# pyxploiter/HandMvNet

Measured on AMD Instinct MI355X. Metric: samples/sec (BxV frames) eval_fps.py, 8-view 256x256; 21-kpt L2 vs reference, higher is better.
Workload: dtype f32; 1 GPU; BASELINE configs[2]: B=32/GPU x V=8 x 256x256, resnet50_paper backbone, d=524, cross_attn x5, GCN decoder; global_batch=32, views=8, frame=256, parallelism=sample-shard x1

## Files before the change

### handmvnet_amd/csrc/conv_igemm.hip

```cpp
#include <cstdio>
#include <cstdlib>
#include <cstring>
#include <type_traits>

#include "kernels.h"

namespace hmv {

typedef float f32x16 __attribute__((ext_vector_type(16)));
typedef float f32x4 __attribute__((ext_vector_type(4)));
typedef _Float16 f16x8 __attribute__((ext_vector_type(8)));
typedef _Float16 f16x4 __attribute__((ext_vector_type(4)));


#ifndef HMV_UB
#define HMV_UB 4
#endif
#ifndef HMV_UB_F16
#define HMV_UB_F16 4
#endif
#ifndef HMV_TOUT
#define HMV_TOUT 1
#endif

// ... 939 lines not shown
                            _Float16 *op = reinterpret_cast<_Float16 *>(outv) + orow[u] * p.ldc + col;
                            if constexpr (W == 8)
                                *reinterpret_cast<f16x8 *>(op) = f16x8{(_Float16)t[0][0], (_Float16)t[0][1], (_Float16)t[0][2], (_Float16)t[0][3],
                                                                       (_Float16)t[W4 - 1][0], (_Float16)t[W4 - 1][1], (_Float16)t[W4 - 1][2], (_Float16)t[W4 - 1][3]};
                            else
                                *reinterpret_cast<f16x4 *>(op) = f16x4{(_Float16)t[0][0], (_Float16)t[0][1], (_Float16)t[0][2], (_Float16)t[0][3]};
                        } else {
#pragma unroll
                            for (int q = 0; q < W4; ++q)
                                *reinterpret_cast<f32x4 *>(reinterpret_cast<float *>(outv) + orow[u] * p.ldc + col + 4 * q) = t[q];
                        }
                    }
                }
            };
            bool wide = false;
            if constexpr (F16 && !GENERIC && BN % 8 == 0 && (NT % (BN / 8)) == 0)
                wide = (p.out_f16 || p.out_split) && ((p.out_split ? p.ldc >> 1 : p.ldc) & 7) == 0 &&
                       (p.res == nullptr || ((p.res_split ? p.ldr >> 1 : p.ldr) & 7) == 0);
            if constexpr (F16 && !GENERIC && BN % 8 == 0 && (NT % (BN / 8)) == 0) {
                if (wide) drain(std::integral_constant<int, 8>{});
                else drain(std::integral_constant<int, 4>{});
            } else {
                drain(std::integral_constant<int, 4>{});
            }
            }
        } else if (GENERIC) {
            for (int idx = tid; idx < SR * BN; idx += NT) {
                const int sr = idx / BN, c = idx - sr * BN;
                const int m = mt * BM + tile_row(sr), col = n0 + c;
                if (m >= p.M || col >= p.Cout) continue;
                const size_t orow = p.scatter ? out_row(m) : (size_t)m;
                const size_t rrow = p.rg_out ? (size_t)(m / p.rg_out) * p.rg_in + (m % p.rg_out) : (size_t)m;
                float v = sC[sr * LDC + c] + p.bias[col];
                if (p.res) v += p.res_f16 ? (float)reinterpret_cast<const _Float16 *>(p.res)[rrow * p.ldr + col]
                                          : reinterpret_cast<const float *>(p.res)[rrow * p.ldr + col];
                if (p.act == ACT_RELU) v = v > 0.f ? v : 0.f;
                else if (p.act == ACT_GELU) v = 0.5f * v * (1.f + erff(v * 0.70710678118654752440f));
                else if (p.act == ACT_LEAKY) v = v > 0.f ? v : 0.01f * v;
                if (p.out_f16) reinterpret_cast<_Float16 *>(outv)[orow * p.ldc + col] = (_Float16)v;
                else reinterpret_cast<float *>(outv)[orow * p.ldc + col] = v;
            }
        }
    }
    if (p.dbg && tid == 0) {
        unsigned hwid, xcc;
        asm volatile("s_getreg_b32 %0, hwreg(HW_REG_HW_ID)" : "=s"(hwid));
        asm volatile("s_getreg_b32 %0, hwreg(HW_REG_XCC_ID)" : "=s"(xcc));
        unsigned long long *d = p.dbg + 8 * (size_t)blockIdx.x;
        d[0] = t1c - t0c; d[1] = t1r - t0r; d[2] = t_entry; d[3] = t0r; d[4] = t1r;
        d[5] = __builtin_amdgcn_s_memrealtime(); d[6] = hwid; d[7] = xcc;
    }
}

int conv_tile_bn(ConvTile t) {
    switch (t) {
        case TILE_128x32: return 32;
        case TILE_128x64: case TILE_64x64: return 64;
        case TILE_128x256: case TILE_256x256: case TILE_128x256_K16: case TILE_256x256_RING: return 256;
        default: return 128;
    }
}

static const char *kTileShape[TILE_COUNT] = {"128x32", "128x64", "128x128", "256x128", "128x256", "256x256", "128x128,k16",
                                              "128x256,k16", "256x128,k16", "64x64", "256x128,k16,w8", "256x256,ring"};
static const char *tile_name(const char *dtype, ConvTile t, int mode, bool partn = false, bool rd = false) {
    static char names[2][TILE_COUNT][3][3][56];
    if (t < 0 || t >= TILE_COUNT || mode < 0 || mode > 2) return "conv_igemm<?>";
    const int d = dtype[1] == '1';
    char *n = names[d][t][mode][rd ? 2 : (partn ? 1 : 0)];
    if (!n[0])
        snprintf(n, sizeof(names[0][0][0][0]), "conv_igemm_%s<%s,%s%s>", dtype, kTileShape[t],
                 mode == 0 ? "taps" : (mode == 1 ? "1x1" : "dense"), rd ? ",rowsum" : (partn ? ",skipN" : ""));
    return n;
}
const char *conv_tile_name_f16(ConvTile t, int mode) {
    return tile_name("f16", t, mode);
}
const char *conv_tile_name(ConvTile t, int mode) { return tile_name("f32", t, mode); }

ConvTile conv_dense_tile(ConvTile t, bool f16) {
    switch (t) {
        case TILE_128x32: case TILE_128x64: case TILE_64x64: case TILE_256x128: return t;
        case TILE_256x128_K16: case TILE_256x256: case TILE_256x256_RING: return TILE_256x128;
        default: return TILE_128x128;
    }
}
bool conv_partial_n(ConvTile t, int Cout) {
    if (t != TILE_128x128 && t != TILE_256x128 && t != TILE_256x256) return false;
    const int bn = conv_tile_bn(t);
    return (Cout + bn - 1) / bn * bn - Cout >= 32;
}

ConvTile conv_pick_tile(int M, int Cout, int K, bool f16, bool has_res) {
    static const int forced = HMV_DEV_INT("HMV_FORCE_TILE", -1);
    static const bool force_all = HMV_DEV_ENV("HMV_FORCE_TILE_ALL") != nullptr;
    if ((Cout > 64 || force_all) && forced >= 0 && forced < TILE_COUNT) return (ConvTile)forced;
    if (!f16 && Cout >= 256 && K <= 128 && M >= 65536) return TILE_128x128_K16;
    static const bool no_w8 = HMV_DEV_ENV("HMV_NO_W8") != nullptr;
    if (!no_w8 && !f16 && has_res && K <= 256 && Cout >= 512 && (long long)((M + 255) / 256) * ((Cout + 127) / 128) >= 2048)
        return TILE_256x128_K16W8;
    if (!no_w8 && !f16 && !has_res && K >= 256 && K <= 512 && Cout == 128 && (long long)((M + 255) / 256) >= 1024)
        return TILE_256x128_K16W8;
    if (!f16 && Cout > 64 && Cout <= 192 && Cout % 64 != 0 && M >= 16384 && K < 2048) return TILE_128x32;
    if (!f16 && Cout > 256 && Cout % 128 != 0 && Cout % 128 <= 64 && M >= 16384 && (long long)((M + 127) / 128) * ((Cout + 63) / 64) < 1024)
        return TILE_64x64;
    if (Cout > 128 && Cout <= 192 && M >= 16384) return (M + 255) / 256 >= 256 ? TILE_256x256 : TILE_128x64;
    if (Cout > 256 && M >= 16384 && Cout % 128 != 0 && Cout % 128 <= 64) return TILE_128x64;
    if (Cout > 128 && (long long)((M + 255) / 256) * ((Cout + 255) / 256) >= 512) return TILE_256x256;
    if (Cout > 64 && (long long)((M + 255) / 256) * ((Cout + 127) / 128) >= 512) return TILE_256x128;
    if (!f16 && K >= 2048 && Cout >= 256 && (long long)((M + 127) / 128) * ((Cout + 127) / 128) < 256 &&
        (long long)((M + 127) / 128) * ((Cout + 63) / 64) >= 256)
        return TILE_128x64;
    if (Cout > 32 && (long long)((M + 127) / 128) * ((Cout + 127) / 128) < 256) return TILE_64x64;
    if (!f16 && K <= 256 && Cout >= 256 && (long long)((M + 127) / 128) * ((Cout + 127) / 128) < 1024) return TILE_64x64;
    if (Cout > 64) return TILE_128x128;
    if (Cout > 32) return TILE_128x64;
    return TILE_128x32;
}

template <typename T, int BM, int BN, int WGM, int WGN, int MODE, bool GENERIC, int KB, bool PARTN = false, bool RD = false, bool X3 = false, bool C32 = false>
static hipError_t launch_one(ConvParams p, hipStream_t s) {
    if constexpr (!X3 && sizeof(T) == 2 && KB == 64 && !GENERIC && !PARTN && !RD && MODE != MODE_HALO) {
        if (p.x3_plane) return launch_one<T, BM, BN, WGM, WGN, MODE, GENERIC, KB, PARTN, RD, true>(p, s);
    }
    constexpr bool tout = HMV_TOUT && sizeof(T) == 2 && !GENERIC && !RD;
    constexpr int ns = ring_stages(sizeof(T) == 2, KB, GENERIC, RD, BM, BN);
    const size_t lds = MODE == MODE_HALO ? (size_t)2 * (HALO_ROWS + BN) * KB * sizeof(T) + 256
                                         : (size_t)lds_floats(BM, BN, WGM, KB * (int)sizeof(T) / 4, RD, !tout, ns) * sizeof(float) + (tout ? 256 : 0);
    auto kern = conv_igemm<T, BM, BN, WGM, WGN, MODE, GENERIC, KB, PARTN, RD, X3, C32>;
    static DeviceOnce once;
    if (const hipError_t e = once.run([&](int) { return set_max_lds(lds, kern); }); e != hipSuccess) return e;
    p.mtiles = (p.M + BM - 1) / BM;
    p.ntiles = (p.Cout + BN - 1) / BN;
    if (p.mtiles * p.ntiles < 4 * p.stagger_blocks) p.stagger = 0;
    hipLaunchKernelGGL(kern, dim3(p.mtiles * p.ntiles * (p.ksl > 1 ? p.ksl : 1) * (p.phases > 1 ? p.phases : 1)), dim3(64 * WGM * WGN), lds, s, p);
    return hipGetLastError();
}

template <typename T, int BM, int BN, int WGM, int WGN, int KB>
static hipError_t launch_modes(const ConvParams &p, bool one, bool generic, hipStream_t s) {
    if (generic) return one ? launch_one<T, BM, BN, WGM, WGN, MODE_1X1, true, KB>(p, s) : launch_one<T, BM, BN, WGM, WGN, MODE_TAPS, true, KB>(p, s);
    return one ? launch_one<T, BM, BN, WGM, WGN, MODE_1X1, false, KB>(p, s) : launch_one<T, BM, BN, WGM, WGN, MODE_TAPS, false, KB>(p, s);
}
template <typename T, int BM, int BN, int WGM, int WGN, int KB>
static hipError_t launch_plain(const ConvParams &p, bool one, hipStream_t s) {
    return one ? launch_one<T, BM, BN, WGM, WGN, MODE_1X1, false, KB>(p, s) : launch_one<T, BM, BN, WGM, WGN, MODE_TAPS, false, KB>(p, s);
}

hipError_t launch_conv(ConvParams p, ConvTile tile, hipStream_t s, const char **name, const ConvRoute &route) {
    if (name) *name = "conv_igemm<none>";
    if (p.M <= 0) return hipSuccess;
    {
        float *page = nullptr;
        hipError_t e = ensure_zero_page(&page);
        if (e != hipSuccess) return e;
        p.zero = page;
    }
    if (!p.lda) p.lda = p.Cin;
    if (!p.ldw) p.ldw = p.Kpad;
    {
        struct Stagger { int ticks = 0, blocks = 256, mode = 0; };
        static const Stagger st = [] {
            Stagger r;
            if (const char *e = HMV_DEV_ENV("HMV_STAGGER")) {
                r.ticks = atoi(e);
                const char *c = strchr(e, ',');
                if (c) { r.blocks = atoi(c + 1); c = strchr(c + 1, ','); if (c) r.mode = atoi(c + 1); }
            }
            return r;
        }();
        p.stagger = st.ticks;
        p.stagger_blocks = st.blocks;
        p.stagger_mode = st.mode;
        static const int pf = HMV_DEV_INT("HMV_PREFETCH", 0);
        p.prefetch = pf;
        static const int burst = HMV_DEV_INT("HMV_BURST", 1);
        p.burst = burst;
    }
    p.acc_scale = ldexpf(1.f, -p.acc_shift);
    bool generic = p.scatter || p.rg_out || p.act == ACT_GELU || p.act == ACT_LEAKY || (p.ldc & 3) ||
                   (p.res && (p.ldr & 3));
    if (HMV_TOUT && p.in_f16 && (p.out_f16 || p.out_split) &&
        (((p.out_split ? p.ldc >> 1 : p.ldc) & 7) || (p.res && ((p.res_split ? p.ldr >> 1 : p.ldr) & 7))))
        generic = true;
    if (p.phases > 1 && (p.phases != 4 || !p.scatter || p.R != 2 || p.S != 2 || p.stride != 1 || p.ksl > 1 || p.in2 || p.rd_cout || p.phase_stride == 0))
        return hipErrorInvalidValue;
    const bool one = p.R == 1 && p.S == 1 && p.pad_h == 0 && p.pad_w == 0;
    if (p.nx_wgt && (generic || p.tall || !conv_stream_chain_ok(p, p.nx_cout, route))) return hipErrorInvalidValue;
    if (p.pool && (generic || p.tall || !conv_hs_supported(p, route))) return hipErrorInvalidValue;
// ... 31 lines not shown
                    tile == TILE_128x256_K16 || tile == TILE_256x128_K16))
        tile = TILE_128x128;
    const int ch = p.in_f16 ? 64 : 32, epc = p.in_f16 ? 8 : 4;
    const bool dense = p.Cin % ch != 0;
    if (p.x3_plane && (!p.in_f16 || generic || p.rd_cout || p.cwrap || p.x3_plane % 8 != 0 || p.Cin != 2 * p.x3_plane ||
                       (!dense && p.x3_plane % 32 != 0) || tile == TILE_128x128_K16 || tile == TILE_128x256_K16 || tile == TILE_256x128_K16 || tile == TILE_256x256_RING))
        return hipErrorInvalidValue;
    if ((p.cwrap || p.res_split || p.out_split || p.acc_shift) &&
        (!p.in_f16 || p.rd_cout || (p.ldc & 3) || (p.res && (p.ldr & 3)) || p.act == ACT_GELU || p.act == ACT_LEAKY))
        return hipErrorInvalidValue;
    if (p.rd_cout && !generic && conv_rds_supported(p, route)) return launch_conv_rds(p, s, name);
    if (p.rd_cout) {
        if (generic || p.R != 3 || p.S != 1 || p.stride != 1 || p.pad_h != 1 || p.pad_w != 0 || p.Cout != 3 * p.rd_cout || p.Cout > 256 ||
            (p.rd_cout & 3) || (p.ldc & 3) || (p.res && (p.ldr & 3)) || 128 % p.Wo != 0 || p.Ho != p.H || p.Wo != p.W)
            return hipErrorInvalidValue;
        if (dense) {
            if (p.Cin % epc != 0 || p.lda % epc != 0 || p.Kpad > (1 << 16)) return hipErrorInvalidValue;
            p.cpt = p.Cin / epc;
            p.cpt_magic = p.cpt > 1 ? (unsigned)(0xFFFFFFFFu / (unsigned)p.cpt) + 1u : 0u;
            p.s_magic = 0u;
        }
        const bool wide = p.Cout > 128;
        if (name) *name = tile_name(p.in_f16 ? "f16" : "f32", wide ? TILE_128x256 : TILE_128x128, dense ? 2 : 0, false, true);
#define HMV_RD(T_, KB_)                                                                                                  \
        if (wide) return dense ? launch_one<T_, 128, 256, 2, 4, MODE_DENSE, false, KB_, false, true>(p, s)                  \
                               : launch_one<T_, 128, 256, 2, 4, MODE_TAPS, false, KB_, false, true>(p, s);                  \
        return dense ? launch_one<T_, 128, 128, 2, 2, MODE_DENSE, false, KB_, false, true>(p, s)                            \
                     : launch_one<T_, 128, 128, 2, 2, MODE_TAPS, false, KB_, false, true>(p, s);
        if (p.in_f16) { HMV_RD(_Float16, 64) }
        HMV_RD(float, 32)
#undef HMV_RD
    }
    if (dense) {
        if (p.Cin % epc != 0 || p.lda % epc != 0 || generic || p.Kpad > (1 << 16)) return hipErrorInvalidValue;
        p.cpt = (p.x3_plane ? p.x3_plane : p.Cin) / epc;
        p.cpt_magic = p.cpt > 1 ? (unsigned)(0xFFFFFFFFu / (unsigned)p.cpt) + 1u : 0u;
        p.s_magic = p.S > 1 ? (unsigned)(0xFFFFFFFFu / (unsigned)p.S) + 1u : 0u;
        if (p.up && (p.R != 1 || p.S != 1 || p.pad_h || p.pad_w || p.stride != 1)) return hipErrorInvalidValue;
        tile = conv_dense_tile(tile, p.in_f16 != 0);
    }
    static const int ring = HMV_DEV_INT("HMV_F16_RING", 0);
    if (ring && p.in_f16 && tile == TILE_256x256 && !generic && !dense && !p.x3_plane && !p.cwrap && !p.rd_cout && p.ksl <= 1)
        tile = TILE_256x256_RING;
    static const bool halo = HMV_DEV_ENV("HMV_NO_HALO") == nullptr;
    const bool use_halo = halo && p.in_f16 && (tile == TILE_256x256 || tile == TILE_256x128) && !generic && !dense && !p.x3_plane && !p.cwrap && !p.rd_cout &&
                          p.ksl <= 1 && !p.in2 && !p.res && !p.up && p.R == 3 && p.S == 3 && p.stride == 1 && p.pad_h == 1 && p.pad_w == 1 &&
                          p.Ho == p.H && p.Wo == p.W && p.H % 16 == 0 && p.W % 16 == 0 && p.Cin % 64 == 0 && p.lda == p.Cin &&
                          p.M % 256 == 0;
    if (use_halo) {
        if (name) *name = tile == TILE_256x256 ? "conv_igemm_f16<256x256,halo>" : "conv_igemm_f16<256x128,halo>";
        return tile == TILE_256x256 ? launch_one<_Float16, 256, 256, 2, 4, MODE_HALO, false, 64>(p, s)
                                    : launch_one<_Float16, 256, 128, 4, 2, MODE_HALO, false, 64>(p, s);
    }
    const int mode = dense ? MODE_DENSE : (one ? MODE_1X1 : MODE_TAPS);
    static const int no_skip = HMV_DEV_INT("HMV_NO_SKIPN", 0);
    const bool partn = !no_skip && !p.in_f16 && !generic && conv_partial_n(tile, p.Cout) && !(dense && tile == TILE_256x256);
    if (name) *name = p.in_f16 ? conv_tile_name_f16(tile, mode) : tile_name("f32", tile, mode, partn);
    if (partn) {
#define HMV_PARTN(BM_, BN_, WGM_, WGN_)                                                                              \
        switch (mode) {                                                                                                 \
            case MODE_DENSE: return launch_one<float, BM_, BN_, WGM_, WGN_, MODE_DENSE, false, 32, true>(p, s);         \
            case MODE_1X1: return launch_one<float, BM_, BN_, WGM_, WGN_, MODE_1X1, false, 32, true>(p, s);             \
            default: return launch_one<float, BM_, BN_, WGM_, WGN_, MODE_TAPS, false, 32, true>(p, s);                  \
        }
        if (tile == TILE_128x128) { HMV_PARTN(128, 128, 2, 2) }
        if (tile == TILE_256x128) { HMV_PARTN(256, 128, 4, 2) }
        if (tile == TILE_256x256) { HMV_PARTN(256, 256, 2, 4) }
#undef HMV_PARTN
    }
    if (dense) {
        if (p.in_f16) {
            static const bool no192 = HMV_DEV_ENV("HMV_NO_N192") != nullptr;
            if (tile == TILE_256x128 && p.Cout > 128 && p.Cout <= 192 && !generic && !no192) {
                if (name) *name = "conv_igemm_f16<256x192,dense>";
                return launch_one<_Float16, 256, 192, 4, 2, MODE_DENSE, false, 64>(p, s);
            }
            switch (tile) {
                case TILE_128x32: return launch_one<_Float16, 128, 32, 4, 1, MODE_DENSE, false, 64>(p, s);
                case TILE_128x64: return launch_one<_Float16, 128, 64, 2, 2, MODE_DENSE, false, 64>(p, s);
                case TILE_64x64: return launch_one<_Float16, 64, 64, 2, 2, MODE_DENSE, false, 64>(p, s);
                case TILE_256x128: return launch_one<_Float16, 256, 128, 4, 2, MODE_DENSE, false, 64>(p, s);
                default: return launch_one<_Float16, 128, 128, 2, 2, MODE_DENSE, false, 64>(p, s);
            }
        }
        switch (tile) {
            case TILE_128x32: return launch_one<float, 128, 32, 4, 1, MODE_DENSE, false, 32>(p, s);
            case TILE_128x64: return launch_one<float, 128, 64, 2, 2, MODE_DENSE, false, 32>(p, s);
            case TILE_64x64: return launch_one<float, 64, 64, 2, 2, MODE_DENSE, false, 32>(p, s);
            case TILE_256x128: return launch_one<float, 256, 128, 4, 2, MODE_DENSE, false, 32>(p, s);
            default: return launch_one<float, 128, 128, 2, 2, MODE_DENSE, false, 32>(p, s);
        }
    }
    if (p.in_f16) {
        switch (tile) {
            case TILE_128x32: return launch_modes<_Float16, 128, 32, 4, 1, 64>(p, one, generic, s);
            case TILE_128x64: return launch_modes<_Float16, 128, 64, 2, 2, 64>(p, one, generic, s);
            case TILE_64x64: return launch_modes<_Float16, 64, 64, 2, 2, 64>(p, one, generic, s);
            case TILE_128x128: return launch_modes<_Float16, 128, 128, 2, 2, 64>(p, one, generic, s);
            case TILE_128x128_K16: return launch_plain<_Float16, 128, 128, 2, 2, 32>(p, one, s);
            case TILE_256x128: return launch_plain<_Float16, 256, 128, 4, 2, 64>(p, one, s);
            case TILE_128x256: return launch_plain<_Float16, 128, 256, 2, 4, 64>(p, one, s);
            case TILE_256x128_K16: return launch_plain<_Float16, 256, 128, 4, 2, 32>(p, one, s);
            case TILE_128x256_K16: return launch_plain<_Float16, 128, 256, 2, 4, 32>(p, one, s);
            case TILE_256x256: return launch_plain<_Float16, 256, 256, 2, 4, 64>(p, one, s);
            case TILE_256x256_RING: return launch_plain<_Float16, 256, 256, 2, 4, 32>(p, one, s);
            default: return hipErrorInvalidValue;
        }
    }
    switch (tile) {
        case TILE_128x32: return launch_modes<float, 128, 32, 4, 1, 32>(p, one, generic, s);
        case TILE_128x64: {
            static const bool no25664 = HMV_DEV_ENV("HMV_NO_T256x64") != nullptr;
            if (!no25664 && !generic && !one && p.Cout == 64 && p.M >= 524288) {
                if (name) *name = "conv_igemm_f32<256x64,taps>";
                return launch_plain<float, 256, 64, 4, 2, 32>(p, false, s);
            }
            return launch_modes<float, 128, 64, 2, 2, 32>(p, one, generic, s);
        }
        case TILE_128x128: return launch_modes<float, 128, 128, 2, 2, 32>(p, one, generic, s);
        case TILE_256x128: return launch_plain<float, 256, 128, 4, 2, 32>(p, one, s);
        case TILE_128x256: return launch_plain<float, 128, 256, 2, 4, 32>(p, one, s);
        case TILE_256x256: return launch_plain<float, 256, 256, 2, 4, 32>(p, one, s);
        case TILE_128x128_K16: return launch_plain<float, 128, 128, 2, 2, 16>(p, one, s);
        case TILE_128x256_K16: return launch_plain<float, 128, 256, 2, 2, 16>(p, one, s);
        case TILE_256x128_K16: return launch_plain<float, 256, 128, 2, 2, 16>(p, one, s);
        case TILE_64x64: return launch_modes<float, 64, 64, 2, 2, 32>(p, one, generic, s);
        case TILE_256x128_K16W8: return launch_plain<float, 256, 128, 4, 2, 16>(p, one, s);
        default: return hipErrorInvalidValue;
    }
}

}
```

### handmvnet_amd/csrc/engine.hip

```cpp
#include <hip/hip_runtime.h>

#include <algorithm>
#include <array>
#include <cmath>
#include <cstdarg>
#include <cstdio>
#include <cstdlib>
#include <cstring>
#include <map>
#include <string>
#include <vector>

#include "../../include/handmv.h"
#include "kernels.h"

using namespace hmv;

namespace {

constexpr int NJ = 21, HEADS = 8, DHEAD = 128, INNER = HEADS * DHEAD;
constexpr int DHEAD_LQ = 256, INNER_LQ = HEADS * DHEAD_LQ;
const int kBlocks[3][4] = {{2, 2, 2, 2}, {3, 4, 6, 3}, {3, 4, 6, 3}};
const int kHrChannels[2][4] = {{40, 80, 160, 320}, {64, 128, 256, 512}};
inline int cpad(int c) { return (c + 3) / 4 * 4; }
// ... 2155 lines not shown
    eng.host["w"] = wt;
    bt.shape = {Cout};
    bt.data.assign(Cout, 0.f);
    if (bias_host) bt.data.assign(bias_host, bias_host + Cout);
    if (rd) {
        HostTensor g1 = bt, m0 = bt, v1 = bt;
        g1.data.assign(Cout, 1.f); m0.data.assign(Cout, 0.f);
        v1.data.assign(Cout, 1.f - 1e-5f);
        eng.host["bn.weight"] = g1; eng.host["bn.bias"] = bt; eng.host["bn.running_mean"] = m0; eng.host["bn.running_var"] = v1;
    } else if (bias_host) {
        eng.host["b"] = bt;
    }
    Loader L{&eng};
    L.split = dtype == HMV_F32X3;
    Layer layer;
    L.conv(layer, "op", "w", bias_host && !rd ? "b" : "", rd ? "bn" : "", Cout, Cin, R, S, 0, half, rd, nullptr, tall);
    int rc = L.rc;
    if (rc == HMV_OK && rd && !layer.rd_cout) { eng.err = "the layer was not packed row-decomposed"; rc = HMV_ERR_ARG; }
    const int Ho = (H + 2 * pad - R) / stride + 1, Wo = (W + 2 * pad - S) / stride + 1;
    const void *x = in, *res = residual;
    void *din = nullptr, *dres = nullptr;
    hipError_t e = hipSuccess;
    if (rc == HMV_OK && half) {
        const int mode = dtype == HMV_F32X3 ? 2 : 1;
        const size_t rows_in = (size_t)N * H * W, rows_out = (size_t)N * Ho * Wo;
        e = hipMalloc(&din, rows_in * Cin * 2 * mode);
        if (e == hipSuccess && residual) e = hipMalloc(&dres, rows_out * Cout * 2 * mode);
        if (e == hipSuccess) e = launch_rows_f32_to_half(in, din, rows_in, Cin, mode, s);
        if (e == hipSuccess && residual) e = launch_rows_f32_to_half(residual, dres, rows_out, Cout, mode, s);
        x = din;
        res = dres;
    }
    if (rc == HMV_OK && e == hipSuccess) {
        Arena dummy;
        Runner Rn{&eng, s, false, HMV_OK, dummy};
        Rn.kernel_name = kernel_name;
        Rn.route = route;
        Rn.conv(layer, static_cast<const float *>(x), N, H, W, stride, pad, pad, static_cast<float *>(out), Cout, static_cast<const float *>(res),
                Cout, relu ? ACT_RELU : ACT_NONE, Ho, Wo, 0, 0, 0, 0, 0, out16);
        rc = Rn.rc;
        if (rc == HMV_OK) e = hipStreamSynchronize(s);
    }
    if (din) (void)hipFree(din);
    if (dres) (void)hipFree(dres);
    for (void *ptr : eng.dev_allocs) (void)hipFree(ptr);
    if (rc != HMV_OK) { g_create_err = std::string(who) + ": " + eng.err; return rc; }
    if (e != hipSuccess) { g_create_err = std::string(who) + ": " + hipGetErrorString(e); return HMV_ERR_HIP; }
    return HMV_OK;
}

static ConvRoute route_sel(int sel) {
    ConvRoute r = conv_rule();
    if (sel) r.stream = sel == 2 ? ROUTE_FORCE : ROUTE_NEVER;
    return r;
}
static ConvRoute route_f16(int sel) {
    ConvRoute r = conv_rule();
    if (sel) r.stream = r.gemm8 = r.hs = (sel == 2 || sel == 8) ? ROUTE_FORCE : ROUTE_NEVER;
    if (sel >= 3 && sel <= 7) r.ht = (sel == 4 || sel == 6) ? ROUTE_NEVER : ROUTE_FORCE;
    r.ht_m16 = sel != 5 && sel != 6;
    r.ht_persist = sel == 7 ? 2 : (sel == 3 ? 0 : 1);
    r.gemm8_persist = sel == 8 ? 2 : (sel == 2 ? 0 : 1);
    return r;
}
static ConvRoute route_x3(int sel) {
    ConvRoute r = conv_rule();
    if (sel) r.x3k16 = sel == 2 ? ROUTE_FORCE : ROUTE_NEVER;
    return r;
}
static ConvRoute route_rd(int sel) {
    ConvRoute r = conv_rule();
    if (sel) r.rds = sel == 2 ? ROUTE_FORCE : ROUTE_NEVER;
    return r;
}

extern "C" {

int hmv_op_conv2d(int32_t device, const float *in, int32_t N, int32_t H, int32_t W, int32_t Cin, const float *w_oihw,
                  const float *bias_host, int32_t Cout, int32_t R, int32_t S, int32_t stride, int32_t pad, const float *residual,
                  int32_t relu, float *out, void *stream) {
    return op_conv("hmv_op_conv2d", device, HMV_F32, in, N, H, W, Cin, w_oihw, bias_host, Cout, R, S, stride, pad, residual, relu, out, false,
                   conv_rule(), nullptr, stream);
}

int hmv_op_conv2d_ex(int32_t device, int32_t dtype, const float *in, int32_t N, int32_t H, int32_t W, int32_t Cin, const float *w_oihw,
                     const float *bias_host, int32_t Cout, int32_t R, int32_t S, int32_t stride, int32_t pad, const float *residual,
                     int32_t relu, float *out, void *stream) {
    return op_conv("hmv_op_conv2d_ex", device, dtype, in, N, H, W, Cin, w_oihw, bias_host, Cout, R, S, stride, pad, residual, relu, out, false,
                   conv_rule(), nullptr, stream);
}

int hmv_op_conv2d_sel(int32_t device, const float *in, int32_t N, int32_t H, int32_t W, int32_t Cin, const float *w_oihw, const float *bias_host,
                      int32_t Cout, int32_t R, int32_t S, int32_t stride, int32_t pad, const float *residual, int32_t relu, float *out,
                      int32_t kernel_sel, const char **kernel_name, void *stream) {
    if (kernel_sel < 0 || kernel_sel > 2) { g_create_err = "hmv_op_conv2d_sel: kernel_sel must be 0, 1 or 2"; return HMV_ERR_ARG; }
    return op_conv("hmv_op_conv2d_sel", device, HMV_F32, in, N, H, W, Cin, w_oihw, bias_host, Cout, R, S, stride, pad, residual, relu, out, false,
                   route_sel(kernel_sel), kernel_name, stream);
}

int hmv_op_conv2d_f16(int32_t device, const float *in, int32_t N, int32_t H, int32_t W, int32_t Cin, const float *w_oihw, const float *bias_host,
                      int32_t Cout, int32_t R, int32_t S, int32_t stride, int32_t pad, const float *residual, int32_t relu, void *out_f16,
                      int32_t kernel_sel, const char **kernel_name, void *stream) {
    if (kernel_sel < 0 || kernel_sel > 8) { g_create_err = "hmv_op_conv2d_f16: kernel_sel must be 0 .. 8"; return HMV_ERR_ARG; }
    return op_conv("hmv_op_conv2d_f16", device, HMV_F16, in, N, H, W, Cin, w_oihw, bias_host, Cout, R, S, stride, pad, residual, relu, out_f16,
                   true, route_f16(kernel_sel), kernel_name, stream, kernel_sel >= 3 && kernel_sel <= 7);
}

int hmv_op_conv2d_x3(int32_t device, const float *in, int32_t N, int32_t H, int32_t W, int32_t Cin, const float *w_oihw, const float *bias_host,
                     int32_t Cout, int32_t R, int32_t S, int32_t stride, int32_t pad, const float *residual, int32_t relu, float *out,
                     int32_t kernel_sel, const char **kernel_name, void *stream) {
    if (kernel_sel < 0 || kernel_sel > 2) { g_create_err = "hmv_op_conv2d_x3: kernel_sel must be 0, 1 or 2"; return HMV_ERR_ARG; }
    return op_conv("hmv_op_conv2d_x3", device, HMV_F32X3, in, N, H, W, Cin, w_oihw, bias_host, Cout, R, S, stride, pad, residual, relu, out, false,
                   route_x3(kernel_sel), kernel_name, stream);
}

int hmv_op_conv2d_rd(int32_t device, const float *in, int32_t N, int32_t H, int32_t W, int32_t C, const float *w_oihw, const float *bias_host,
                     const float *residual, int32_t relu, float *out, int32_t kernel_sel, const char **kernel_name, void *stream) {
    if (!in || !w_oihw || !out || C % 4 != 0 || 3 * C > 256 || C % 32 == 0 || W <= 0 || 128 % W != 0 || kernel_sel < 0 || kernel_sel > 2) {
        g_create_err = "hmv_op_conv2d_rd: C % 4 == 0, C % 32 != 0, 3 C <= 256, 128 % W == 0, kernel_sel 0 .. 2";
        return HMV_ERR_ARG;
    }
    return op_conv("hmv_op_conv2d_rd", device, HMV_F32, in, N, H, W, C, w_oihw, bias_host, C, 3, 3, 1, 1, residual, relu, out, false,
                   route_rd(kernel_sel), kernel_name, stream, false, true);
}

}

extern "C" int hmv_op_hr_fuse_up(int32_t device, int32_t f16, const float *base, int32_t N, int32_t H, int32_t W, int32_t C, int32_t nsrc,
                                 const float *const *src, const int32_t *src_c, const int32_t *shift, const float *const *w_host,
                                 const float *const *bias_host, int32_t relu, void *out, void *stream) {
    if (!base || !out || !src || !src_c || !shift || !w_host || !bias_host || nsrc < 1 || nsrc > 3 || N <= 0 || H <= 0 || W <= 0 || C <= 0) {
        g_create_err = "hmv_op_hr_fuse_up: bad arguments";
        return HMV_ERR_ARG;
    }
    if (hipSetDevice(device) != hipSuccess) { g_create_err = "hipSetDevice failed"; return HMV_ERR_HIP; }
    hipStream_t s = static_cast<hipStream_t>(stream);
    HrFuseParams p{};
    p.N = N; p.H = H; p.W = W; p.C = C; p.ldc = C; p.nsrc = nsrc; p.relu = relu ? 1 : 0; p.f16 = f16 ? 1 : 0;
    std::vector<void *> owned;
    auto fail = [&](int rc, const std::string &msg) {
        for (void *q : owned) (void)hipFree(q);
        g_create_err = "hmv_op_hr_fuse_up: " + msg;
        return rc;
    };
    hipError_t e = hipSuccess;
    auto dev_copy = [&](const std::vector<float> &v) -> float * {
        void *d = nullptr;
        if (e == hipSuccess) e = hipMalloc(&d, v.size() * sizeof(float));
// ... 34 lines not shown
```

### handmvnet_amd/csrc/kernels.h

```cpp
#pragma once
#include <hip/hip_runtime.h>
#include <stdint.h>
#include <stdlib.h>

#include <atomic>
#include <mutex>

#ifdef HMV_DEV_KNOBS
#define HMV_DEV_ENV(name) getenv(name)
#else
#define HMV_DEV_ENV(name) (static_cast<const char *>(nullptr))
#endif
#define HMV_DEV_INT(name, dflt) (HMV_DEV_ENV(name) ? atoi(HMV_DEV_ENV(name)) : (dflt))

namespace hmv {

enum Act { ACT_NONE = 0, ACT_RELU = 1, ACT_GELU = 2, ACT_LEAKY = 3 };

class DeviceOnce {
    std::atomic<bool> done_[64] = {};
    std::mutex m_;
public:
    template <typename F>
    hipError_t run(F &&body, int *dev_out = nullptr) {
// ... 35 lines not shown
    int scatter;
    int osy, osx, ooy, oox;
    int mtiles, ntiles;
    const float *zero;
    int cpt;
    unsigned cpt_magic, s_magic;
    int cwrap;
    int res_split;
    int x3_plane;
    int acc_shift;
    float acc_scale;
    int out_split;
    int ngroup;
    int m16;
    int tall;
    int rd_cout;
    const void *in2;
    int ksplit, H2, W2, lda2, stride2;
    int lda;
    int ldw;
    int ksl, kslice;
    size_t out_slice;
    int phases;
    size_t phase_stride;
    int burst;
    int prefetch;
    int stagger;
    int stagger_mode;
    int stagger_blocks;
    unsigned long long *dbg;
    int pool, pool_h, pool_w;
    const void *nx_wgt;
    const float *nx_bias;
    void *nx_out;
    int nx_cout, nx_ldw, nx_ldc, nx_act;
};

enum ConvTile { TILE_128x32 = 0, TILE_128x64 = 1, TILE_128x128 = 2, TILE_256x128 = 3, TILE_128x256 = 4, TILE_256x256 = 5,
                TILE_128x128_K16 = 6, TILE_128x256_K16 = 7, TILE_256x128_K16 = 8, TILE_64x64 = 9,
                TILE_256x128_K16W8 = 10,
                TILE_256x256_RING = 11,
                TILE_COUNT = 12 };
int conv_tile_bn(ConvTile t);
const char *conv_tile_name(ConvTile t, int mode);
const char *conv_tile_name_f16(ConvTile t, int mode);
ConvTile conv_pick_tile(int M, int Cout, int K, bool f16 = false, bool has_res = false);
ConvTile conv_dense_tile(ConvTile t, bool f16);
bool conv_partial_n(ConvTile t, int Cout);

enum { ROUTE_RULE = -1, ROUTE_NEVER = 0, ROUTE_FORCE = 1 };
struct ConvRoute {
    int stream = ROUTE_RULE, gemm8 = ROUTE_RULE, hs = ROUTE_RULE, rds = ROUTE_RULE, ht = ROUTE_RULE, x3k16 = ROUTE_RULE;
    int gemm8_persist = 1, ht_persist = 1;
    int ht_m16 = 1;
};
inline const ConvRoute &conv_rule() {
    static const ConvRoute r = [] {
        ConvRoute q;
        if (HMV_DEV_ENV("HMV_NO_STREAM")) q.stream = ROUTE_NEVER;
        if (HMV_DEV_ENV("HMV_NO_GEMM8")) q.gemm8 = ROUTE_NEVER;
        if (HMV_DEV_ENV("HMV_NO_HS")) q.hs = ROUTE_NEVER;
        if (HMV_DEV_ENV("HMV_NO_RDS")) q.rds = ROUTE_NEVER;
        return q;
    }();
    return r;
}

hipError_t launch_conv(ConvParams p, ConvTile tile, hipStream_t s, const char **name = nullptr, const ConvRoute &route = conv_rule());
bool conv_stream_supported(const ConvParams &p, const ConvRoute &route = conv_rule());
bool conv_stream_chain_ok(const ConvParams &p, int nx_cout, const ConvRoute &route = conv_rule());
hipError_t launch_conv_stream(const ConvParams &p, hipStream_t s, const char **name);

hipError_t launch_nchw_to_nhwc4(const float *x, float *out, int N, int H, int W, hipStream_t s);
hipError_t launch_maxpool3s2(const float *in, float *out, int N, int H, int W, int C, int Ho, int Wo, hipStream_t s);
hipError_t launch_soft_argmax(const float *hm, int ld, int N, int h, int w, float *coords, float *crop_img,
                              float image_size, float heatmap_size, float *hm_nchw, hipStream_t s);
hipError_t launch_sample_gather(const float *feat, int N, int H, int W, int C, const float *coords, float *out,
                                hipStream_t s, int elem_bytes = 4);
hipError_t launch_nchw_to_nhwc8_f16(const float *x, void *out, int N, int H, int W, hipStream_t s);
hipError_t launch_frames_to_input(const uint8_t *frames, const int *boxes, int N, int Hf, int Wf, int S_h, int S_w, const float *mean,
                                  const float *std, int out_mode, void *out, hipStream_t s, bool s2d = false);
hipError_t launch_nchw_to_s2d(const float *x, void *out, int N, int H, int W, int mode, hipStream_t s);
hipError_t launch_nchw_to_nhwc_split(const float *x, void *out, int N, int H, int W, hipStream_t s);
hipError_t launch_maxpool3s2_split(const void *in, void *out, int N, int H, int W, int C, int Ho, int Wo, hipStream_t s);
hipError_t launch_nhwc_split_to_nchw(const void *in, float *out, int N, int H, int W, int C, hipStream_t s);
hipError_t launch_rows_f32_to_half(const float *in, void *out, size_t rows, int C, int mode, hipStream_t s);
hipError_t launch_maxpool3s2_f16(const void *in, void *out, int N, int H, int W, int C, int Ho, int Wo, hipStream_t s);
hipError_t launch_nhwc_f16_to_nchw(const void *in, float *out, int N, int H, int W, int C, hipStream_t s);
hipError_t launch_sample_blend(const float *s4, int lds4, int C, int N, int H, int W, const float *coords,
                               float *tokens, int ldt, int col0, hipStream_t s);
hipError_t launch_tokens_finalize(float *tokens, int ldt, int d, int fdim, int N, int V, const float *coords,
                                  const float *bbox, const float *intr, int pos_mask, const float *pe,
                                  float *raw_copy, hipStream_t s, void *pairs = nullptr);
hipError_t launch_layernorm(const float *x, int ldx, int rows, int d, const float *g1, const float *b1, float *y,
                            int ldy, const float *g2, const float *b2, float *y2, hipStream_t s);
hipError_t launch_attention(const float *qkv, int B, int T, int Tq, int koff, int Tk, float *out, hipStream_t s, int pairs = 0, int x3 = 0);
hipError_t launch_attention_d256(const float *q, int q_ld, int q_bstride, const float *k, const float *v, int kv_ld, int B, int T,
                                 int Tq, float *out, hipStream_t s, int pairs = 0);
hipError_t launch_add_pe(const float *x, int ldx, int rows, int T, int d, const float *pe, float *y, int ldy, hipStream_t s);
hipError_t launch_splitk_layernorm(const float *slab, int S, int rows, int lds, int d, const float *bias, const float *res, int ldr,
                                   int rg_out, int rg_in, const float *g1, const float *b1, float *y, int ldy, const float *g2,
                                   const float *b2, float *y2, hipStream_t s);
hipError_t launch_splitk_reduce(const float *slab, int S, int rows, int lds, int N, const float *bias, const float *res, int ldr,
                                int rg_out, int rg_in, int act, float *out, int ldc, hipStream_t s);
hipError_t launch_cheb_mix(const float *y, int ldy, int B, int co, const float *tk, const float *bias, int leaky,
                           float *out, int ldo, hipStream_t s);
// ... 59 lines not shown
```

Baseline: 6023 frames/s.

## Add persistent f32 256x256 implicit-GEMM conv kernel with epilogue/prologue overlap

Adds a persistent-grid f32 256x256 implicit-GEMM conv kernel launched with at most one block per CU. Blocks walk tiles in an XCD-aware order and start the next tile's global-to-LDS loads before storing the last epilogue pass of the current tile. It replaces the plain 256x256 f32 launch when the shape qualifies, there is no residual, and there are at least twice as many tiles as CUs. The aim is to hide per-tile prologue and epilogue latency and cut block launch overhead, at the cost of more complex wait-count logic and possible load imbalance when tiles do not divide evenly across CUs.

```diff
diff --git a/handmvnet_amd/csrc/conv_igemm.hip b/handmvnet_amd/csrc/conv_igemm.hip
--- a/handmvnet_amd/csrc/conv_igemm.hip
+++ b/handmvnet_amd/csrc/conv_igemm.hip
@@ -1015,6 +1015,240 @@
     }
 }
 
+template <int MODE>
+__global__ __launch_bounds__(512, 2) void conv_igemm32p(const ConvParams p) {
+    constexpr int BM = 256, BN = 256, WGM = 2, WGN = 4, KB = 32, NT = 64 * WGM * WGN;
+    constexpr int LPR = KB / 4, RPW = 64 / LPR, RPS = NT / LPR, NQ = LPR / 2;
+    constexpr int WM = BM / WGM, WN = BN / WGN, TM = WM / 32, TN = WN / 32, AP = BM / RPS, BP = BN / RPS, LDC = BN + 4;
+    constexpr int AS = stage_blocks(BM, BN, WGM, KB), SR = WGM * AS * 32, NPS = TM / AS;
+    constexpr int TPR = BN / 4, RPP = NT / TPR, NPASS = SR / RPP;
+    constexpr int NST = NPASS;
+    static_assert(MODE == MODE_1X1 || MODE == MODE_TAPS, "chunked modes");
+    static_assert(TM % AS == 0 && SR * LDC <= lds_floats(BM, BN, WGM, KB) && SR % RPP == 0 && AP + BP + NST < 64, "epilogue shape / vmcnt range");
+    extern __shared__ __attribute__((aligned(16))) float smem[];
+    float *sA = smem, *sB = smem + 2 * BM * KB;
+
+    const int tid = threadIdx.x, lane = tid & 63;
+    const int wave = __builtin_amdgcn_readfirstlane(tid >> 6);
+    const int l31 = lane & 31, kh = lane >> 5;
+    const int wm = wave / WGN, wn = wave % WGN;
+    const int lrow = tid / LPR, kqs = (tid & 7) ^ ((tid >> 4) & 7), koff = 4 * kqs;
+    const float *zero = p.zero;
+    const int HoWo = p.Ho * p.Wo, nk = p.Kpad / KB, ntile = p.mtiles * p.ntiles;
+    auto tile_of = [&](int v, int &mt_, int &nt_) {
+        const int xcd = v & 7, loc = v >> 3, q = ntile >> 3, r = ntile & 7;
+        const int lid = (xcd < r ? xcd * (q + 1) : r * (q + 1) + (xcd - r) * q) + loc;
+        mt_ = lid / p.ntiles;
+        nt_ = lid - mt_ * p.ntiles;
+    };
+
+    const float *aptr[AP], *wptr[BP];
+    int astep[AP], hi0[AP], wi0[AP];
+    int dmt = 0, cr = 0, cs = 0, cc = 0, cdelta = 0, ck = 0;
+    auto setup = [&](int mt_, int nt_) {
+        dmt = mt_;
+        cr = cs = cc = cdelta = ck = 0;
+#pragma unroll
+        for (int i = 0; i < AP; ++i) {
+            const int m = mt_ * BM + i * RPS + lrow;
+            const bool ok = m < p.M;
+            const int mm = ok ? m : 0;
+            const int n = mm / HoWo, rem = mm - n * HoWo;
+            const int ho = rem / p.Wo, wo = rem - ho * p.Wo;
+            const float *base = reinterpret_cast<const float *>(p.in) + (size_t)n * p.H * p.W * p.lda;
+            hi0[i] = ok ? ho * p.stride - p.pad_h : -(1 << 28);
+            wi0[i] = wo * p.stride - p.pad_w;
+            if constexpr (MODE == MODE_1X1) {
+                aptr[i] = ok ? base + (hi0[i] * p.W + wi0[i]) * p.lda + koff : zero;
+                astep[i] = ok ? KB : 0;
+            } else {
+                aptr[i] = base + (ok ? (hi0[i] * p.W + wi0[i]) * p.lda + koff : 0);
+                astep[i] = 0;
+            }
+        }
+#pragma unroll
+        for (int i = 0; i < BP; ++i) wptr[i] = reinterpret_cast<const float *>(p.wgt) + (size_t)(nt_ * BN + i * RPS + lrow) * p.ldw + 4 * kqs;
+    };
+#define HMV_P_DMA(buf)                                                                                      \
+    {                                                                                                       \
+        _Pragma("unroll") for (int i = 0; i < AP; ++i) {                                                    \
+            const float *src_;                                                                              \
+            if constexpr (MODE == MODE_1X1) {                                                               \
+                src_ = aptr[i];                                                                             \
+                aptr[i] += astep[i];                                                                        \
+            } else {                                                                                        \
+                const bool ok_ = (unsigned)(hi0[i] + cr) < (unsigned)p.H && (unsigned)(wi0[i] + cs) < (unsigned)p.W; \
+                src_ = ok_ ? aptr[i] + cdelta : zero;                                                       \
+            }                                                                                               \
+            HMV_GLDS16(src_, sA + ((buf) * BM + i * RPS + wave * RPW) * KB);                                \
+        }                                                                                                   \
+        _Pragma("unroll") for (int i = 0; i < BP; ++i) {                                                    \
+            HMV_GLDS16(wptr[i], sB + ((buf) * BN + i * RPS + wave * RPW) * KB);                             \
+            wptr[i] += KB;                                                                                  \
+        }                                                                                                   \
+        ck += KB;                                                                                           \
+        if (MODE == MODE_1X1 && p.in2 && ck == p.ksplit) {  \
+            _Pragma("unroll") for (int i = 0; i < AP; ++i) {                                                \
+                const int m_ = dmt * BM + i * RPS + lrow;                                                   \
+                if (m_ < p.M) {                                                                             \
+                    const int n_ = m_ / HoWo, rem_ = m_ - n_ * HoWo, ho_ = rem_ / p.Wo, wo_ = rem_ - ho_ * p.Wo; \
+                    aptr[i] = reinterpret_cast<const float *>(p.in2) + ((size_t)n_ * p.H2 * p.W2 +          \
+                              (size_t)(ho_ * p.stride2) * p.W2 + wo_ * p.stride2) * p.lda2 + koff;          \
+                }                                                                                           \
+            }                                                                                               \
+        }                                                                                                   \
+        if (MODE == MODE_TAPS) {                       \
+            cdelta += p.lda;                                                                                \
+            if (++cs == p.S) {                                                                              \
+                cs = 0;                                                                                     \
+                cdelta += (p.W - p.S) * p.lda;                                                              \
+                if (++cr == p.R) { cr = 0; cc += KB; cdelta = cc; }                                         \
+            }                                                                                               \
+        }                                                                                                   \
+    }
+    const int fsw = (l31 >> 1) & 7;
+    const float *arow = sA + (wm * WM + l31) * KB, *brow = sB + (wn * WN + l31) * KB;
+#define HMV_P_FRAGS(FA, FB, buf, q)                                                                         \
+    {                                                                                                       \
+        const int ch_ = ((2 * (q) + kh) ^ fsw) * 4;                                                         \
+        _Pragma("unroll") for (int a = 0; a < TM; ++a)                                                      \
+            FA[a] = *reinterpret_cast<const f32x4 *>(arow + ((buf) * BM + a * 32) * KB + ch_);              \
+        _Pragma("unroll") for (int b = 0; b < TN; ++b)                                                      \
+            FB[b] = *reinterpret_cast<const f32x4 *>(brow + ((buf) * BN + b * 32) * KB + ch_);              \
+    }
+#define HMV_P_MFMA(FA, FB)                                                                                  \
+    {                                                                                                       \
+        _Pragma("unroll") for (int e = 0; e < 4; ++e)                                                       \
+            _Pragma("unroll") for (int a = 0; a < TM; ++a)                                                  \
+                _Pragma("unroll") for (int b = 0; b < TN; ++b)                                              \
+                    acc[a][b] = __builtin_amdgcn_mfma_f32_32x32x2f32(FA[a][e], FB[b][e], acc[a][b], 0, 0, 0); \
+    }
+
+    int v = blockIdx.x, mt, nt;
+    tile_of(v, mt, nt);
+    unsigned long long t_start = p.dbg ? __builtin_amdgcn_s_memrealtime() : 0;
+    setup(mt, nt);
+    HMV_P_DMA(0);
+    HMV_P_DMA(1);
+    asm volatile("s_waitcnt vmcnt(%0)\n\ts_barrier" ::"n"(AP + BP) : "memory");
+    bool pend = false;
+    for (;;) {
+        f32x16 acc[TM][TN];
+#pragma unroll
+        for (int a = 0; a < TM; ++a)
+#pragma unroll
+            for (int b = 0; b < TN; ++b)
+#pragma unroll
+                for (int e = 0; e < 16; ++e) acc[a][b][e] = 0.f;
+        f32x4 fa0[TM], fb0[TN], fa1[TM], fb1[TN];
+        unsigned long long t0c = 0, t0r = 0, t1c = 0, t1r = 0;
+        if (p.dbg) { t0c = __builtin_amdgcn_s_memtime(); t0r = __builtin_amdgcn_s_memrealtime(); }
+        HMV_P_FRAGS(fa0, fb0, 0, 0);
+        for (int kt = 0; kt < nk; ++kt) {
+            const int buf = kt & 1;
+#pragma unroll
+            for (int q = 0; q < NQ; ++q) {
+                if (q + 1 < NQ) {
+                    if (q & 1) { HMV_P_FRAGS(fa0, fb0, buf, q + 1); } else { HMV_P_FRAGS(fa1, fb1, buf, q + 1); }
+                } else {
+                    if (kt == 0 && pend) asm volatile("s_waitcnt vmcnt(%0) lgkmcnt(0)\n\ts_barrier" ::"n"(NST) : "memory");
+                    else asm volatile("s_waitcnt vmcnt(0) lgkmcnt(0)\n\ts_barrier" ::: "memory");
+                    if (kt + 2 < nk) HMV_P_DMA(buf);
+                    if (kt + 1 < nk) HMV_P_FRAGS(fa0, fb0, buf ^ 1, 0);
+                }
+                if (q & 1) { HMV_P_MFMA(fa1, fb1); } else { HMV_P_MFMA(fa0, fb0); }
+                __builtin_amdgcn_sched_barrier(0);
+            }
+        }
+        if (p.dbg) { t1c = __builtin_amdgcn_s_memtime(); t1r = __builtin_amdgcn_s_memrealtime(); }
+        asm volatile("s_waitcnt vmcnt(0) lgkmcnt(0)\n\ts_barrier" ::: "memory");
+
+        float *sC = smem;
+        const int c4 = tid % TPR, r0 = tid / TPR, col = nt * BN + 4 * c4;
+        const int cend = (p.fill || p.Cout + 3 >= p.ldc) ? p.ldc : ((p.Cout + 3) & ~3);
+        const bool cok = col < cend;
+        const f32x4 bv = cok ? *reinterpret_cast<const f32x4 *>(p.bias + col) : f32x4{0.f, 0.f, 0.f, 0.f};
+        const bool has_res = p.res != nullptr;
+        const float lo = (p.act == ACT_RELU) ? 0.f : -INFINITY;
+        auto out_m = [&](int ps, int u) {
+            const int sr = r0 + u * RPP;
+            return mt * BM + (sr / (AS * 32)) * WM + (ps * AS + (sr / 32) % AS) * 32 + (sr & 31);
+        };
+        float *trash = const_cast<float *>(p.zero) + 64 + 4 * lane;
+        f32x4 ov[NPASS];
+#pragma unroll
+        for (int ps = 0; ps < NPS; ++ps) {
+            if (ps > 0) asm volatile("s_waitcnt lgkmcnt(0)\n\ts_barrier" ::: "memory");
+#pragma unroll
+            for (int aa = 0; aa < AS; ++aa)
+#pragma unroll
+                for (int b = 0; b < TN; ++b)
+#pragma unroll
+                    for (int e = 0; e < 16; ++e) {
+                        const int srow = (wm * AS + aa) * 32 + (e & 3) + 8 * (e >> 2) + 4 * kh;
+                        sC[srow * LDC + wn * WN + b * 32 + l31] = acc[ps * AS + aa][b][e];
+                    }
+            asm volatile("s_waitcnt lgkmcnt(0)\n\ts_barrier" ::: "memory");
+            auto read_back = [&](auto res_tag) {
+                constexpr bool RES = decltype(res_tag)::value;
+#pragma unroll
+                for (int u = 0; u < NPASS; ++u) {
+                    const int m = out_m(ps, u);
+                    f32x4 rv = {0.f, 0.f, 0.f, 0.f};
+                    if constexpr (RES)
+                        rv = *reinterpret_cast<const f32x4 *>((m < p.M && cok) ? reinterpret_cast<const float *>(p.res) + (size_t)m * p.ldr + col : zero);
+                    f32x4 t = *reinterpret_cast<const f32x4 *>(&sC[(r0 + u * RPP) * LDC + 4 * c4]) + bv + rv;
+#pragma unroll
+                    for (int j = 0; j < 4; ++j) t[j] = fmaxf(t[j], lo);
+                    if (ps + 1 < NPS) {
+                        if (m < p.M && cok) *reinterpret_cast<f32x4 *>(reinterpret_cast<float *>(p.out) + (size_t)m * p.ldc + col) = t;
+                    } else {
+                        ov[u] = t;
+                    }
+                }
+            };
+            if (has_res) read_back(std::true_type{});
+            else read_back(std::false_type{});
+        }
+        asm volatile("s_waitcnt lgkmcnt(0)\n\ts_barrier" ::: "memory");
+
+        const int vn = v + (int)gridDim.x;
+        const bool more = vn < ntile;
+        int mtn = 0, ntn = 0;
+        unsigned long long t_next = 0;
+        if (more) {
+            tile_of(vn, mtn, ntn);
+            if (p.dbg) t_next = __builtin_amdgcn_s_memrealtime();
+            setup(mtn, ntn);
+            HMV_P_DMA(0);
+            HMV_P_DMA(1);
+        }
+        __builtin_amdgcn_sched_barrier(0);
+#pragma unroll
+        for (int u = 0; u < NPASS; ++u) {
+            const int m = out_m(NPS - 1, u);
+            float *dst = (m < p.M && cok) ? reinterpret_cast<float *>(p.out) + (size_t)m * p.ldc + col : trash;
+            *reinterpret_cast<f32x4 *>(dst) = ov[u];
+        }
+        __builtin_amdgcn_sched_barrier(0);
+        if (p.dbg && tid == 0) {
+            unsigned hwid, xcc;
+            asm volatile("s_getreg_b32 %0, hwreg(HW_REG_HW_ID)" : "=s"(hwid));
+            asm volatile("s_getreg_b32 %0, hwreg(HW_REG_XCC_ID)" : "=s"(xcc));
+            unsigned long long *d = p.dbg + 8 * (size_t)v;
+            d[0] = t1c - t0c; d[1] = t1r - t0r; d[2] = t_start; d[3] = t0r; d[4] = t1r;
+            d[5] = __builtin_amdgcn_s_memrealtime(); d[6] = hwid; d[7] = xcc;
+        }
+        if (!more) break;
+        asm volatile("s_waitcnt vmcnt(%0)\n\ts_barrier" ::"n"(AP + BP + NST) : "memory");
+        v = vn; mt = mtn; nt = ntn; t_start = t_next;
+        pend = true;
+    }
+#undef HMV_P_DMA
+#undef HMV_P_FRAGS
+#undef HMV_P_MFMA
+}
+
 int conv_tile_bn(ConvTile t) {
     switch (t) {
         case TILE_128x32: return 32;
@@ -1098,6 +1332,35 @@
     if (p.mtiles * p.ntiles < 4 * p.stagger_blocks) p.stagger = 0;
     hipLaunchKernelGGL(kern, dim3(p.mtiles * p.ntiles * (p.ksl > 1 ? p.ksl : 1) * (p.phases > 1 ? p.phases : 1)), dim3(64 * WGM * WGN), lds, s, p);
     return hipGetLastError();
+}
+
+constexpr size_t kIgemm32pLds = (size_t)lds_floats(256, 256, 2, 32) * sizeof(float);
+static hipError_t igemm32p_cus(int *cus) {
+    static DeviceOnce once;
+    static int ncu[64] = {};
+    int dev = 0;
+    const hipError_t e = once.run([](int d) {
+        hipDeviceProp_t prop;
+        if (hipGetDeviceProperties(&prop, d) != hipSuccess) return hipErrorInvalidDevice;
+        ncu[d] = prop.multiProcessorCount > 0 ? prop.multiProcessorCount : 256;
+        return set_max_lds(kIgemm32pLds, conv_igemm32p<MODE_TAPS>, conv_igemm32p<MODE_1X1>);
+    }, &dev);
+    if (e == hipSuccess) *cus = ncu[dev];
+    return e;
+}
+static hipError_t launch_igemm32p(ConvParams p, bool one, int cus, hipStream_t s, const char **name) {
+    constexpr size_t lds = kIgemm32pLds;
+    p.mtiles = (p.M + 255) / 256;
+    p.ntiles = (p.Cout + 255) / 256;
+    const int tiles = p.mtiles * p.ntiles, grid = tiles < cus ? tiles : cus;
+    if (name) *name = one ? "conv_igemm_f32<256x256,1x1,persistent>" : "conv_igemm_f32<256x256,taps,persistent>";
+    if (one) hipLaunchKernelGGL(conv_igemm32p<MODE_1X1>, dim3(grid), dim3(512), lds, s, p);
+    else hipLaunchKernelGGL(conv_igemm32p<MODE_TAPS>, dim3(grid), dim3(512), lds, s, p);
+    return hipGetLastError();
+}
+static bool igemm32p_shape_ok(const ConvParams &p) {
+    return !p.in_f16 && !p.out_f16 && !p.res_f16 && !p.out_split && !p.res_split && !p.cwrap && !p.x3_plane && !p.acc_shift && !p.rd_cout &&
+           !p.up && p.ksl <= 1 && p.phases <= 1 && p.Kpad >= 64 && p.Kpad % 32 == 0 && p.Cin % 32 == 0;
 }
 
 template <typename T, int BM, int BN, int WGM, int WGN, int KB>
@@ -1235,6 +1498,7 @@
         return tile == TILE_256x256 ? launch_one<_Float16, 256, 256, 2, 4, MODE_HALO, false, 64>(p, s)
                                     : launch_one<_Float16, 256, 128, 4, 2, MODE_HALO, false, 64>(p, s);
     }
+    if (route.igemm32_persist == 2 && !generic && !dense && igemm32p_shape_ok(p) && !conv_partial_n(TILE_256x256, p.Cout)) tile = TILE_256x256;
     const int mode = dense ? MODE_DENSE : (one ? MODE_1X1 : MODE_TAPS);
     static const int no_skip = HMV_DEV_INT("HMV_NO_SKIPN", 0);
     const bool partn = !no_skip && !p.in_f16 && !generic && conv_partial_n(tile, p.Cout) && !(dense && tile == TILE_256x256);
@@ -1303,7 +1567,15 @@
         case TILE_128x128: return launch_modes<float, 128, 128, 2, 2, 32>(p, one, generic, s);
         case TILE_256x128: return launch_plain<float, 256, 128, 4, 2, 32>(p, one, s);
         case TILE_128x256: return launch_plain<float, 128, 256, 2, 4, 32>(p, one, s);
-        case TILE_256x256: return launch_plain<float, 256, 256, 2, 4, 32>(p, one, s);
+        case TILE_256x256: {
+            if (route.igemm32_persist && igemm32p_shape_ok(p)) {
+                int cus = 0;
+                if (const hipError_t e = igemm32p_cus(&cus); e != hipSuccess) return e;
+                if (route.igemm32_persist == 2 || (!p.res && (long long)((p.M + 255) / 256) * ((p.Cout + 255) / 256) >= 2ll * cus))
+                    return launch_igemm32p(p, one, cus, s, name);
+            }
+            return launch_plain<float, 256, 256, 2, 4, 32>(p, one, s);
+        }
         case TILE_128x128_K16: return launch_plain<float, 128, 128, 2, 2, 16>(p, one, s);
         case TILE_128x256_K16: return launch_plain<float, 128, 256, 2, 2, 16>(p, one, s);
         case TILE_256x128_K16: return launch_plain<float, 256, 128, 2, 2, 16>(p, one, s);
diff --git a/handmvnet_amd/csrc/engine.hip b/handmvnet_amd/csrc/engine.hip
--- a/handmvnet_amd/csrc/engine.hip
+++ b/handmvnet_amd/csrc/engine.hip
@@ -2231,6 +2231,7 @@
 static ConvRoute route_sel(int sel) {
     ConvRoute r = conv_rule();
     if (sel) r.stream = sel == 2 ? ROUTE_FORCE : ROUTE_NEVER;
+    if (sel == 1 || sel == 3) r.igemm32_persist = sel == 3 ? 2 : 0;
     return r;
 }
 static ConvRoute route_f16(int sel) {
@@ -2272,7 +2273,7 @@
 int hmv_op_conv2d_sel(int32_t device, const float *in, int32_t N, int32_t H, int32_t W, int32_t Cin, const float *w_oihw, const float *bias_host,
                       int32_t Cout, int32_t R, int32_t S, int32_t stride, int32_t pad, const float *residual, int32_t relu, float *out,
                       int32_t kernel_sel, const char **kernel_name, void *stream) {
-    if (kernel_sel < 0 || kernel_sel > 2) { g_create_err = "hmv_op_conv2d_sel: kernel_sel must be 0, 1 or 2"; return HMV_ERR_ARG; }
+    if (kernel_sel < 0 || kernel_sel > 3) { g_create_err = "hmv_op_conv2d_sel: kernel_sel must be 0 .. 3"; return HMV_ERR_ARG; }
     return op_conv("hmv_op_conv2d_sel", device, HMV_F32, in, N, H, W, Cin, w_oihw, bias_host, Cout, R, S, stride, pad, residual, relu, out, false,
                    route_sel(kernel_sel), kernel_name, stream);
 }
diff --git a/handmvnet_amd/csrc/kernels.h b/handmvnet_amd/csrc/kernels.h
--- a/handmvnet_amd/csrc/kernels.h
+++ b/handmvnet_amd/csrc/kernels.h
@@ -111,6 +111,7 @@
 struct ConvRoute {
     int stream = ROUTE_RULE, gemm8 = ROUTE_RULE, hs = ROUTE_RULE, rds = ROUTE_RULE, ht = ROUTE_RULE, x3k16 = ROUTE_RULE;
     int gemm8_persist = 1, ht_persist = 1;
+    int igemm32_persist = 1;
     int ht_m16 = 1;
 };
 inline const ConvRoute &conv_rule() {
```

Result: no change. 6050 frames/s (median of 6 runs) (+0.4%).
